# ChanTsune/Portable-Network-Archive

Measured on AMD Instinct MI355X. Metric: archive-create MiB/s (input bytes/sec), zstd-3, 10000 x 1 MiB enwik-style corpus, higher is better.
Workload: dtype u8

## Files before the change

portable-network-archive_amd/csrc/k_entropy.hip:

```cpp
#include <hip/hip_runtime.h>
#include "pna_dev.h"

namespace pna {

__constant__ uint8_t C_LL_CODE[64] = {0,1,2,3,4,5,6,7,8,9,10,11,12,13,14,15,16,16,17,17,18,18,19,19,20,20,20,20,21,21,21,21,
                                      22,22,22,22,22,22,22,22,23,23,23,23,23,23,23,23,24,24,24,24,24,24,24,24,24,24,24,24,24,24,24,24};
__constant__ uint8_t C_ML_CODE[128] = {0,1,2,3,4,5,6,7,8,9,10,11,12,13,14,15,16,17,18,19,20,21,22,23,24,25,26,27,28,29,30,31,
                                       32,32,33,33,34,34,35,35,36,36,36,36,37,37,37,37,38,38,38,38,38,38,38,38,39,39,39,39,39,39,39,39,
                                       40,40,40,40,40,40,40,40,40,40,40,40,40,40,40,40,41,41,41,41,41,41,41,41,41,41,41,41,41,41,41,41,
                                       42,42,42,42,42,42,42,42,42,42,42,42,42,42,42,42,42,42,42,42,42,42,42,42,42,42,42,42,42,42,42,42};
__constant__ uint32_t C_LL_BASE[36] = {0,1,2,3,4,5,6,7,8,9,10,11,12,13,14,15,16,18,20,22,24,28,32,40,48,64,128,256,512,1024,2048,4096,8192,16384,32768,65536};
__constant__ uint8_t  C_LL_BITS[36] = {0,0,0,0,0,0,0,0,0,0,0,0,0,0,0,0,1,1,1,1,2,2,3,3,4,6,7,8,9,10,11,12,13,14,15,16};
__constant__ uint32_t C_ML_BASE[53] = {3,4,5,6,7,8,9,10,11,12,13,14,15,16,17,18,19,20,21,22,23,24,25,26,27,28,29,30,31,32,33,34,35,37,39,41,43,47,51,59,67,83,99,131,259,515,1027,2051,4099,8195,16387,32771,65539};
__constant__ uint8_t  C_ML_BITS[53] = {0,0,0,0,0,0,0,0,0,0,0,0,0,0,0,0,0,0,0,0,0,0,0,0,0,0,0,0,0,0,0,0,1,1,1,1,2,2,3,3,4,4,5,7,8,9,10,11,12,13,14,15,16};
__constant__ int16_t C_LL_DEF[36] = {4,3,2,2,2,2,2,2,2,2,2,2,2,1,1,1,2,2,2,2,2,2,2,2,2,3,2,1,1,1,1,1,-1,-1,-1,-1};
__constant__ int16_t C_ML_DEF[53] = {1,4,3,2,2,2,2,2,2,1,1,1,1,1,1,1,1,1,1,1,1,1,1,1,1,1,1,1,1,1,1,1,1,1,1,1,1,1,1,1,1,1,1,1,1,1,-1,-1,-1,-1,-1,-1,-1};
__constant__ int16_t C_OF_DEF[29] = {1,1,1,1,1,1,2,2,2,1,1,1,1,1,1,1,1,1,1,1,1,1,1,1,-1,-1,-1,-1,-1};

__device__ __forceinline__ uint32_t hb(uint32_t v) { return 31u - (uint32_t)__builtin_clz(v); }
__device__ __forceinline__ uint32_t ll_code(uint32_t v) { return v < 64 ? C_LL_CODE[v] : hb(v) + 19; }
__device__ __forceinline__ uint32_t ml_code(uint32_t ml) { uint32_t b = ml - 3; return b < 128 ? C_ML_CODE[b] : hb(b) + 36; }

struct BitW { uint8_t *p; uint32_t pos; uint64_t acc; uint32_t nb; };
__device__ __forceinline__ void bw_init(BitW &w, uint8_t *p) { w.p = p; w.pos = 0; w.acc = 0; w.nb = 0; }
// ... 421 lines not shown
            }
        }
        for (uint32_t j = (n16 << 4) + tid; j < nlit; j += ST_THREADS) atomicAdd(&hl[bl[j]], 1u);
        const uint64_t *bs = seqs + (size_t)g * seq_cap_of(sd.blk_log);
        for (uint32_t i = tid; i < (PRE ? 0u : nseq); i += ST_THREADS) {
            const uint64_t s = bs[i];
            const uint32_t llv = seq_ll(s), mb = seq_ml(s) - 3;
            atomicAdd(&h_seq[0][tid & (HS - 1)][llv < 64 ? (uint32_t)s_llc[llv] : hb(llv) + 19], 1u);
            atomicAdd(&h_seq[1][tid & (HS - 1)][hb(seq_off(s) + 3)], 1u);
            atomicAdd(&h_seq[2][tid & (HS - 1)][mb < 128 ? (uint32_t)s_mlc[mb] : hb(mb) + 36], 1u);
        }
    }
    __syncthreads();
    if (PRE == 1) {
        const uint32_t *hs = hist + (size_t)blockIdx.x * HIST_WORDS;
        count[tid] = hs[tid];
        if (tid < 192) scount[tid >> 6][tid & 63] = hs[256 + tid];
        __syncthreads();
        for (uint32_t s = 0; s < 36; s++) nseq_seg += scount[0][s];
    } else if (PRE == 2) {
        const uint32_t *hs = hist + (size_t)blockIdx.x * HIST_WORDS;
        { uint32_t c = 0; for (uint32_t k = 0; k < HL; k++) c += h_lit[k][tid]; count[tid] = c; }
        if (tid < 192) scount[tid >> 6][tid & 63] = hs[256 + tid];
    } else {
        { uint32_t c = 0; for (uint32_t k = 0; k < HL; k++) c += h_lit[k][tid]; count[tid] = c; }
        if (tid < 192) { uint32_t w = tid >> 6, s = tid & 63, c = 0; for (uint32_t k = 0; k < HS; k++) c += h_seq[w][k][s]; scount[w][s] = c; }
    }
    __syncthreads();
    const uint32_t wave = tid >> 6, lane = tid & 63;
    if (wave != 0) {
        if (!nseq_seg) return;
        bool ok;
        if (wave == 1) ok = seq_build_wave(T, 0, scount[0], nseq_seg, 36, C_LL_DEF, 36, 6, flags, cell[1], tmp192[1], sq_sh[1], lane);
        else if (wave == 2) ok = seq_build_wave(T, 1, scount[1], nseq_seg, 32, C_OF_DEF, 29, 5, flags, cell[2], tmp192[2], sq_sh[2], lane);
        else ok = seq_build_wave(T, 2, scount[2], nseq_seg, 53, C_ML_DEF, 53, 6, flags, cell[3], tmp192[3], sq_sh[3], lane);
        if (!ok && lane == 0) atomicAnd(&T->seq_ok, 0u);
        return;
    }
    if (!(flags & F_HUF)) return;
    const int np = huf_build_lens(count, lens, order, wt, parent, hsh, lane);
    if (np < 2) return;
    uint32_t ms = 0, mb = 0;
    for (int s2 = (int)lane; s2 < 256; s2 += 64) { if (count[s2]) ms = (uint32_t)s2; const uint32_t l = lens[s2]; mb = l > mb ? l : mb; }
#pragma unroll
    for (int o = 32; o > 0; o >>= 1) { const uint32_t a2 = (uint32_t)__shfl_xor((int)ms, o), b2 = (uint32_t)__shfl_xor((int)mb, o); ms = a2 > ms ? a2 : ms; mb = b2 > mb ? b2 : mb; }
    const int max_sym = (int)ms, maxbits = (int)mb;
    if (lane < HUF_MAX + 2) { cntw_s[lane] = 0; crun_s[lane] = 0; }
    __builtin_amdgcn_wave_barrier();
    for (int s2 = (int)lane; s2 < 256; s2 += 64) { const uint32_t l = lens[s2]; if (l && s2 <= max_sym) atomicAdd(&cntw_s[(uint32_t)maxbits + 1 - l], 1u); }
    __builtin_amdgcn_wave_barrier();
    if (lane == 0) {
        uint32_t pos = 0;
        for (int w = 1; w <= maxbits; w++) { wbase_s[w] = pos; pos += cntw_s[w] << (w - 1); }
        hsh[3] = (uint32_t)max_sym; hsh[4] = (uint32_t)maxbits;
    }
    __builtin_amdgcn_wave_barrier();
    const uint64_t lane_lt = ((uint64_t)1 << lane) - 1;
    for (int r = 0; r < 4; r++) {
        const int s2 = 64 * r + (int)lane;
        const uint32_t l = (s2 <= max_sym) ? (uint32_t)lens[s2] : 0u;
        uint32_t before = 0;
        for (uint32_t L = 1; L <= (uint32_t)maxbits; L++) {
            const uint64_t m = __ballot(l == L);
            if (l == L) before = crun_s[L] + (uint32_t)__popcll(m & lane_lt);
            __builtin_amdgcn_wave_barrier();
            if (lane == 0 && m) crun_s[L] += (uint32_t)__popcll(m);
            __builtin_amdgcn_wave_barrier();
        }
        uint32_t v = 0;
        if (l) {
            const uint32_t w = (uint32_t)maxbits + 1 - l;
            v = ((wbase_s[w] + (before << (w - 1))) >> (w - 1)) | (l << 16);
        }
        T->huf_code[s2] = v;
    }
    __builtin_amdgcn_wave_barrier();
    const uint32_t tl = huf_write_tree_wave(T->tree, lens, max_sym, maxbits, wts, tmp, &wtab, cell[0], tmp192[0], sq_sh[0], lane);
    if (lane == 0) { T->tree_len = tl; T->max_sym = (uint32_t)max_sym; T->maxbits = (uint32_t)maxbits; T->huf_ok = tl > 0; }
}

constexpr uint32_t LIT_THREADS = 256;
constexpr uint32_t LIT_STAGE_Q = 184;

__global__ __launch_bounds__(LIT_THREADS)
void k_lit(const SegDesc *__restrict__ segs, const uint32_t *__restrict__ blk_seg, const uint8_t *__restrict__ lits,
           BlkInfo *__restrict__ blk, const SegTables *__restrict__ tabs, uint8_t *__restrict__ litc, uint32_t flags, uint32_t g0, uint32_t blk_log) {
    __shared__ uint32_t code[256];
    __shared__ uint32_t sbits[4];
    __shared__ unsigned long long stage[4][LIT_STAGE_Q];
    const uint32_t tid = threadIdx.x, lane = tid & 63, wave = tid >> 6;
    const uint32_t g = blockIdx.x + g0;
    const SegTables *T = tabs + blk_seg[g];
    const uint32_t nlit = blk[g].nlit;
    const uint8_t *bl = lits + ((size_t)g << blk_log);
    const uint4 *bl16 = (const uint4 *)bl;
    unsigned long long *out64 = (unsigned long long *)(litc + ((size_t)g << blk_log));
    if (!(flags & F_HUF) || nlit < 64) { if (tid == 0) { blk[g].lit_body = 0; blk[g].lit_rle = 0; } return; }
    if (!T->huf_ok) {
        const uint32_t b0 = bl[0] * 0x01010101u; int same = 1;
        const uint32_t n16 = nlit >> 4;
        for (uint32_t i = tid; i < n16; i += LIT_THREADS) { const uint4 v = bl16[i]; same &= (v.x == b0) & (v.y == b0) & (v.z == b0) & (v.w == b0); }
        for (uint32_t i = (n16 << 4) + tid; i < nlit; i += LIT_THREADS) same &= (bl[i] == (uint8_t)b0);
        same = __syncthreads_and(same);
        if (tid == 0) { blk[g].lit_rle = same ? 1u : 0u; blk[g].lit_body = 0; }
        return;
    }
    code[tid] = T->huf_code[tid];
    __syncthreads();
    const uint32_t nstreams = nlit >= 256 ? 4u : 1u;
    const uint32_t segsz = nstreams == 4 ? (nlit + 3) / 4 : nlit;
    const uint32_t a = wave * segsz;
    uint32_t m = 0;
    if (wave < nstreams) m = (nstreams == 4 && wave == 3) ? nlit - 3 * segsz : segsz;
    const uint32_t e = a + m;
    const uint32_t gfirst = a >> 4, gend = m ? (e + 15) >> 4 : gfirst;
    {
        const uint32_t b0 = bl[0];
        uint32_t bits = 0; int same = 1;
        for (uint32_t gi = gfirst + lane; gi < gend; gi += 64) {
            const uint4 v = bl16[gi];
            const uint32_t w[4] = {v.x, v.y, v.z, v.w}, base = gi << 4;
#pragma unroll
            for (uint32_t k = 0; k < 16; k++) {
                const uint32_t i = base + k, sym = (w[k >> 2] >> (8 * (k & 3))) & 0xFF;
                if (i >= a && i < e) { bits += code[sym] >> 16; same &= (sym == b0); }
            }
        }
#pragma unroll
        for (int d = 32; d >= 1; d >>= 1) bits += (uint32_t)__shfl_xor((int)bits, d);
        if (lane == 0) sbits[wave] = wave < nstreams ? bits : 0;
        same = __syncthreads_and(same);
        if (same) { if (tid == 0) { blk[g].lit_rle = 1; blk[g].lit_body = 0; } return; }
    }
    uint32_t sz[4], off[4], body = nstreams == 4 ? 6u : 0u;
    for (uint32_t k = 0; k < 4; k++) { sz[k] = k < nstreams ? (sbits[k] >> 3) + 1 : 0; off[k] = body; body += sz[k]; }
    if (tid == 0) { blk[g].lit_body = body; blk[g].lit_rle = 0; }
    if (body >= nlit || body > (1u << blk_log)) return;
    for (uint32_t i = tid; i < (body + 7) / 8; i += LIT_THREADS) out64[i] = 0;
    for (uint32_t i = lane; i < LIT_STAGE_Q; i += 64) stage[wave][i] = 0;
    __builtin_amdgcn_s_waitcnt(0);
    __syncthreads();
    if (wave < nstreams) {
        unsigned long long *st = stage[wave];
        uint32_t pos = off[wave] * 8;
        uint32_t qfl = pos >> 6;
        const uint32_t nround = (gend - gfirst + 63) / 64;
        for (uint32_t r = 0; r < nround; r++) {
            const int32_t gi = (int32_t)gend - 64 * (int32_t)(r + 1) + (int32_t)lane;
            const bool act = gi >= (int32_t)gfirst;
            unsigned long long gv[4] = {0, 0, 0, 0}; uint32_t gl[4] = {0, 0, 0, 0};
            if (act) {
                const uint4 v = bl16[gi];
                const uint32_t w[4] = {v.x, v.y, v.z, v.w}, base = (uint32_t)gi << 4;
#pragma unroll
                for (int k = 15; k >= 0; k--) {
                    const uint32_t i = base + (uint32_t)k;
                    if (i >= a && i < e) {
                        const uint32_t cv = code[(w[k >> 2] >> (8 * (k & 3))) & 0xFF];
                        const int grp = 3 - (k >> 2);
                        gv[grp] |= (unsigned long long)(cv & 0xFFFF) << gl[grp]; gl[grp] += cv >> 16;
                    }
                }
            }
            const uint32_t ltot = gl[0] + gl[1] + gl[2] + gl[3];
            uint32_t sc = ltot;
#pragma unroll
            for (int d = 1; d < 64; d <<= 1) { uint32_t t = (uint32_t)__shfl_up((int)sc, d); if (lane >= (uint32_t)d) sc += t; }
            const uint32_t rtot = (uint32_t)__shfl((int)sc, 63);
            uint32_t p = pos + (rtot - sc) - (qfl << 6);
#pragma unroll
            for (int grp = 0; grp < 4; grp++) {
                if (gl[grp]) {
                    const uint32_t qi = p >> 6, sh = p & 63;
                    atomicOr(&st[qi], gv[grp] << sh);
                    if (sh + gl[grp] > 64) atomicOr(&st[qi + 1], gv[grp] >> (64 - sh));
                    p += gl[grp];
                }
            }
            pos += rtot;
            const uint32_t nq = (pos >> 6) - qfl;
            const unsigned long long part = st[nq];
            for (uint32_t j = lane; j < nq; j += 64) { const unsigned long long x = st[j]; if (x) atomicOr(&out64[qfl + j], x); }
            for (uint32_t j = lane; j <= nq; j += 64) st[j] = (j == 0) ? part : 0ull;
            qfl += nq;
        }
        if (lane == 0) atomicOr(&st[(pos - (qfl << 6)) >> 6], 1ull << ((pos - (qfl << 6)) & 63));
        pos += 1;
        const uint32_t nq = ((pos - (qfl << 6)) + 63) >> 6;
        for (uint32_t j = lane; j < nq; j += 64) { const unsigned long long x = st[j]; if (x) atomicOr(&out64[qfl + j], x); }
    }
    if (tid == 0 && nstreams == 4) atomicOr(&out64[0], (unsigned long long)sz[0] | ((unsigned long long)sz[1] << 16) | ((unsigned long long)sz[2] << 32));
}

constexpr uint32_t SEQ_SEGS_PER_WG = 64 / BLK_PER_SEG;
static_assert(SEQ_MAX_LOG <= 8, "k_seqa: a state flush is at most 8 bits (12 are kept), the final states go into 3 x 8 bits");

constexpr uint32_t SEQA_BLKS = 21, SEQA_MAXSEG = 5;
__global__ __launch_bounds__(64)
void k_seqa(const SegDesc *__restrict__ segs, uint32_t nseg, BlkInfo *__restrict__ blk, const SegTables *__restrict__ tabs,
            uint16_t *__restrict__ seqw, uint32_t bps_log) {
    __shared__ SeqTable tab[SEQA_MAXSEG][3];
    __shared__ SeqTable ztab;
    const uint32_t lane = threadIdx.x;
    const uint32_t vb0 = blockIdx.x * SEQA_BLKS;
    const uint32_t seg0 = vb0 >> bps_log, seg1 = (vb0 + SEQA_BLKS - 1) >> bps_log;
    for (uint32_t i = lane; i < sizeof(SeqTable) / 4; i += 64) ((uint32_t *)&ztab)[i] = 0;
    for (uint32_t s = seg0; s <= seg1 && s < nseg && s - seg0 < SEQA_MAXSEG; s++) {
        const uint32_t *srcw = (const uint32_t *)&tabs[s].tab[0];
        uint32_t *dstw = (uint32_t *)&tab[s - seg0][0];
        for (uint32_t i = lane; i < 3 * sizeof(SeqTable) / 4; i += 64) dstw[i] = srcw[i];
    }
    __syncthreads();
    const uint32_t slot = lane / 3, st = lane - 3 * slot;
    const uint32_t vb = vb0 + slot;
    const uint32_t sidx = vb >> bps_log, b = vb & ((1u << bps_log) - 1);
    if (lane >= 3 * SEQA_BLKS || sidx >= nseg) return;
    const SegDesc sd = segs[sidx];
    if (b >= seg_nblk(sd)) return;
    const uint32_t g = sd.blk_base + b;
    const SegTables *T = tabs + sidx;
    const uint32_t nseq = blk[g].nseq;
    if (nseq == 0 || !T->seq_ok) { if (st == 0) blk[g].seq_bits = 0; return; }
    const uint32_t mode = T->mode[st], tlog = T->tlog[st];
    const SeqTable *tb = mode == 1 ? &ztab : &tab[sidx - seg0][st];
    const uint32_t SC = seq_cap_of(sd.blk_log);
    uint16_t *w = seqw + (size_t)g * SC * 4 + (size_t)st * SC;
    uint32_t state = 0, bits = 0;
    uint4 *w8 = (uint4 *)w;
    int32_t j = (int32_t)((nseq - 1) >> 3);
    uint4 cur = w8[j], r1 = cur, r2 = cur, r3 = cur;
    if (j > 0) r1 = w8[j - 1];
    if (j > 1) r2 = w8[j - 2];
    if (j > 2) r3 = w8[j - 3];
    bool first = true;
    for (; j >= 0; j--) {
        uint4 r4 = r3;
        if (j > 3) r4 = w8[j - 4];
        const uint32_t cw32[4] = {cur.x, cur.y, cur.z, cur.w};
        uint32_t out[4] = {0, 0, 0, 0};
        const int32_t top = (int32_t)(nseq - 1) - 8 * j;
#pragma unroll
        for (int k = 7; k >= 0; k--) {
            if (k > top) continue;
            const uint32_t cw = (cw32[k >> 1] >> (16 * (k & 1))) & 0xFFFFu;
            const SeqSym y = tb->sym[cw & 0xFF];
            uint32_t rec = 0;
            if (first) { state = y.first_state; first = false; }
            else {
                const uint32_t nb = (state + y.delta_nb) >> 16;
                rec = (state & ((1u << nb) - 1)) | (nb << 12);
                state = tb->state[(int)(state >> nb) + y.delta_find];
                bits += nb;
            }
            bits += cw >> 8;
            out[k >> 1] |= rec << (16 * (k & 1));
        }
        w8[j] = make_uint4(out[0], out[1], out[2], out[3]);
        cur = r1; r1 = r2; r2 = r3; r3 = r4;
    }
    bits += mode != 1 ? tlog : 0u;
    const uint32_t b1 = (uint32_t)__shfl((int)bits, (int)(3 * slot + 1)), b2 = (uint32_t)__shfl((int)bits, (int)(3 * slot + 2));
    atomicOr(&blk[g].pad, (state & ((1u << tlog) - 1)) << (st == 2 ? 0 : (st == 1 ? 8 : 16)));
    if (st == 0) blk[g].seq_bits = (bits + b1 + b2 + 1 + 7) >> 3;
}

template <bool GT>
__global__ __launch_bounds__(64)
void k_seq(const SegDesc *__restrict__ segs, uint32_t nseg, const uint64_t *__restrict__ seqs, BlkInfo *__restrict__ blk,
           const SegTables *__restrict__ tabs, uint8_t *__restrict__ seqc, uint32_t bps_log) {
    __shared__ SeqTable tab[GT ? 1 : SEQ_SEGS_PER_WG][3];
    __shared__ SeqTable ztab;
    __shared__ uint32_t lut_ll[64], lut_ml[128];
    __shared__ uint32_t ring[8][64];
// ... 266 lines not shown
        for (int d = 1; d < 64; d <<= 1) { const uint32_t t = (uint32_t)__shfl_up((int)incl, d); if ((int)lane >= d) incl += t; }
        if (in) { blk[g].plan = plan; blk[g].out_size = sz; blk[g].out_off = off + (incl - sz); }
        off += (uint32_t)__shfl((int)incl, 63);
    }
    if (lane == 0) seg_size[sidx] = off;
}

__global__ __launch_bounds__(1024)
void k_scan(const uint64_t *__restrict__ in, uint64_t *__restrict__ out, uint32_t n) {
    __shared__ uint64_t part[2][1024];
    const uint32_t tid = threadIdx.x;
    const uint32_t per = (n + 1023) / 1024;
    const uint32_t a = tid * per, e = a + per < n ? a + per : n;
    uint64_t s = 0;
    for (uint32_t i = a; i < e; i++) s += in[i];
    uint32_t cur = 0;
    part[0][tid] = s;
    __syncthreads();
    const uint32_t nact = per ? (n + per - 1) / per : 0;
    for (uint32_t d = 1; d < 1024 && d < nact; d <<= 1) {
        const uint64_t v = part[cur][tid] + (tid >= d ? part[cur][tid - d] : 0ull);
        part[cur ^ 1][tid] = v;
        cur ^= 1;
        __syncthreads();
    }
    uint64_t r = part[cur][tid] - s;
    if (tid == 0) out[n] = nact ? part[cur][nact - 1] : 0ull;
    for (uint32_t i = a; i < e; i++) { out[i] = r; r += in[i]; }
}

constexpr uint32_t WR_THREADS = 256;
typedef uint32_t wr_v4u __attribute__((ext_vector_type(4)));
__device__ __forceinline__ void copy_bytes(uint8_t *dst, const uint8_t *src, uint32_t n, uint32_t tid, uint32_t T) {
    const uint32_t head = (uint32_t)((16u - ((uintptr_t)dst & 15u)) & 15u), h = head < n ? head : n, mid = (n - h) >> 4;
    if (tid < h) dst[tid] = src[tid];
    for (uint32_t i = tid; i < mid; i += T) { wr_v4u v; __builtin_memcpy(&v, src + h + 16 * i, 16); *(wr_v4u *)(dst + h + 16 * i) = v; }
    for (uint32_t i = h + 16 * mid + tid; i < n; i += T) dst[i] = src[i];
}

__global__ __launch_bounds__(WR_THREADS)
void k_write(const uint8_t *__restrict__ src, const SegDesc *__restrict__ segs, const uint32_t *__restrict__ blk_seg,
             const BlkInfo *__restrict__ blk, const SegTables *__restrict__ tabs, const uint64_t *__restrict__ seg_off,
             const uint8_t *__restrict__ lits, const uint8_t *__restrict__ litc, const uint8_t *__restrict__ seqc,
             uint8_t *__restrict__ dst) {
    const uint32_t tid = threadIdx.x, g = blockIdx.x, NT = blockDim.x;
    const uint32_t sidx = blk_seg[g];
    const SegDesc sd = segs[sidx];
    const SegTables *T = tabs + sidx;
    const BlkInfo bi = blk[g];
    const uint32_t b = g - sd.blk_base;
    const uint32_t nblk = seg_nblk(sd), bsz = 1u << sd.blk_log;
    const uint32_t b0 = b * bsz, bl_len = sd.len - b0 < bsz ? sd.len - b0 : bsz;
    const bool single = (sd.first & 4) != 0;
    const uint32_t last = (b + 1 == nblk && (!single || (sd.first & 2))) ? 1u : 0u;
    uint8_t *fr = dst + seg_off[sidx];
    uint8_t *out = fr + bi.out_off;
    if (b == 0 && tid < 6 && (!single || (sd.first & 1))) { const uint8_t fh[6] = {0x28, 0xB5, 0x2F, 0xFD, 0x00, 0x50}; fr[tid] = fh[tid]; }
    const uint32_t csz = bi.out_size - 3;
    if (tid < 3) { uint32_t hdr = last | ((bi.plan & 1 ? 2u : 0u) << 1) | (csz << 3); out[tid] = (uint8_t)(hdr >> (8 * tid)); }
    out += 3;
    if (!(bi.plan & 1)) { copy_bytes(out, src + sd.src_off + b0, bl_len, tid, NT); return; }
    const uint32_t nlit = bi.nlit, nseq = bi.nseq;
    const uint8_t *bl = lits + ((size_t)g << sd.blk_log);
    uint32_t pos = 0;
    if (bi.plan & 16) {
        uint32_t h = raw_lit_hdr(nlit);
        if (tid == 0) {
            if (h == 1) out[0] = (uint8_t)(1 | (nlit << 3));
            else if (h == 2) { out[0] = (uint8_t)(1 | (1 << 2) | ((nlit & 15) << 4)); out[1] = (uint8_t)(nlit >> 4); }
            else { out[0] = (uint8_t)(1 | (3 << 2) | ((nlit & 15) << 4)); out[1] = (uint8_t)(nlit >> 4); out[2] = (uint8_t)(nlit >> 12); }
            out[h] = bl[0];
        }
        pos = h + 1;
    } else if (bi.plan & 2) {
        const uint32_t lh = 3 + (nlit >= 1024) + (nlit >= 16384), ts = (bi.plan & 4) ? T->tree_len : 0, hs = bi.lit_body;
        if (tid == 0) {
            uint64_t type = (bi.plan & 4) ? 2u : 3u, comp = ts + hs, h;
            if (lh == 3) h = type | ((uint64_t)(nlit >= 256 ? 1 : 0) << 2) | ((uint64_t)nlit << 4) | (comp << 14);
            else if (lh == 4) h = type | (2u << 2) | ((uint64_t)nlit << 4) | (comp << 18);
            else h = type | (3u << 2) | ((uint64_t)nlit << 4) | (comp << 22);
            for (uint32_t i = 0; i < lh; i++) out[i] = (uint8_t)(h >> (8 * i));
        }
        copy_bytes(out + lh, T->tree, ts, tid, NT);
        copy_bytes(out + lh + ts, litc + ((size_t)g << sd.blk_log), hs, tid, NT);
        pos = lh + ts + hs;
    } else {
        uint32_t h = raw_lit_hdr(nlit);
        if (tid == 0) {
            if (h == 1) out[0] = (uint8_t)(nlit << 3);
            else if (h == 2) { out[0] = (uint8_t)((1 << 2) | ((nlit & 15) << 4)); out[1] = (uint8_t)(nlit >> 4); }
            else { out[0] = (uint8_t)((3 << 2) | ((nlit & 15) << 4)); out[1] = (uint8_t)(nlit >> 4); out[2] = (uint8_t)(nlit >> 12); }
        }
        copy_bytes(out + h, bl, nlit, tid, NT);
        pos = h + nlit;
    }
    const uint32_t nh = nseq_hdr(nseq);
    if (tid == 0) {
        if (nh == 1) out[pos] = (uint8_t)nseq;
        else if (nh == 2) { out[pos] = (uint8_t)((nseq >> 8) + 128); out[pos + 1] = (uint8_t)nseq; }
        else { out[pos] = 255; out[pos + 1] = (uint8_t)(nseq - 0x7F00); out[pos + 2] = (uint8_t)((nseq - 0x7F00) >> 8); }
    }
    pos += nh;
    if (nseq) {
        const bool carry = (bi.plan & 8) != 0;
        if (tid == 0) {
            uint32_t m[3];
            for (int k = 0; k < 3; k++) m[k] = T->mode[k] == 0 ? 0u : (carry ? T->mode[k] : 3u);
            out[pos] = (uint8_t)((m[0] << 6) | (m[1] << 4) | (m[2] << 2));
        }
        pos += 1;
        if (carry) for (int k = 0; k < 3; k++) { copy_bytes(out + pos, T->desc[k], T->desc_len[k], tid, NT); pos += T->desc_len[k]; }
        copy_bytes(out + pos, seqc + ((size_t)g << sd.blk_log), bi.seq_bits, tid, NT);
    }
}

__global__ void k_empty(const SegDesc *__restrict__ segs, uint32_t nseg, const uint64_t *__restrict__ seg_off, uint8_t *__restrict__ dst) {
    const uint32_t sidx = blockIdx.x * blockDim.x + threadIdx.x;
    if (sidx >= nseg || segs[sidx].len != 0) return;
    const uint8_t e[9] = {0x28, 0xB5, 0x2F, 0xFD, 0x20, 0x00, 0x01, 0x00, 0x00};
    uint8_t *o = dst + seg_off[sidx];
    for (int i = 0; i < 9; i++) o[i] = e[i];
}

__global__ __launch_bounds__(1024)
void k_scan_a(const uint64_t *__restrict__ in, uint64_t *__restrict__ out, uint32_t n, uint64_t *__restrict__ chunk_sum) {
    __shared__ uint64_t part[2][1024];
    const uint32_t tid = threadIdx.x, i0 = blockIdx.x * 4096 + tid * 4;
    uint64_t v[4], s = 0;
#pragma unroll
    for (uint32_t k = 0; k < 4; k++) { v[k] = i0 + k < n ? in[i0 + k] : 0ull; s += v[k]; }
    uint32_t cur = 0;
    part[0][tid] = s;
    __syncthreads();
    for (uint32_t d = 1; d < 1024; d <<= 1) {
        part[cur ^ 1][tid] = part[cur][tid] + (tid >= d ? part[cur][tid - d] : 0ull);
        cur ^= 1;
        __syncthreads();
    }
    uint64_t r = part[cur][tid] - s;
#pragma unroll
    for (uint32_t k = 0; k < 4; k++) { if (i0 + k < n) out[i0 + k] = r; r += v[k]; }
    if (tid == 1023) chunk_sum[blockIdx.x] = part[cur][1023];
}
__global__ __launch_bounds__(1024)
void k_scan_c(uint64_t *__restrict__ out, uint32_t n, const uint64_t *__restrict__ chunk_off, uint32_t nchunk) {
    const uint32_t i0 = blockIdx.x * 4096 + threadIdx.x * 4;
    const uint64_t o = chunk_off[blockIdx.x];
#pragma unroll
    for (uint32_t k = 0; k < 4; k++) if (i0 + k < n) out[i0 + k] += o;
    if (blockIdx.x == 0 && threadIdx.x == 0) out[n] = chunk_off[nchunk];
}
void k_scan_launch(const uint64_t *in, uint64_t *out, uint32_t n, hipStream_t st) {
    hipLaunchKernelGGL(k_scan, dim3(1), dim3(1024), 0, st, in, out, n);
}
void k_scan_launch_big(const uint64_t *in, uint64_t *out, uint32_t n, hipStream_t st) {
    if (n <= 65536) { k_scan_launch(in, out, n, st); return; }
    const uint32_t nchunk = (n + 4095) / 4096;
    uint64_t *chunk_sum = out + n + 1, *chunk_off = chunk_sum + nchunk + 1;
    hipLaunchKernelGGL(k_scan_a, dim3(nchunk), dim3(1024), 0, st, in, out, n, chunk_sum);
    hipLaunchKernelGGL(k_scan, dim3(1), dim3(1024), 0, st, chunk_sum, chunk_off, nchunk);
    hipLaunchKernelGGL(k_scan_c, dim3(nchunk), dim3(1024), 0, st, out, n, chunk_off, nchunk);
}

void launch_entropy_chunk(const SegDesc *segs, uint32_t s0, uint32_t ns, const uint32_t *blk_seg, uint32_t g0, uint32_t nb,
                          const uint64_t *seqs, const uint8_t *lits, BlkInfo *blk, SegTables *tabs, uint8_t *litc, uint8_t *seqc, uint32_t *seqw,
                          uint32_t flags, uint32_t blk_log, uint32_t *hist, hipStream_t st, hipEvent_t *ev ,
                          hipStream_t side, hipEvent_t fork, hipEvent_t join, bool single_block , const uint32_t *seq_hist) {
// ... 52 lines not shown
```

portable-network-archive_amd/csrc/pna_dev.h:

```cpp
#pragma once
#include <stdint.h>
#include <stddef.h>
#include "aes_core.h"

namespace pna {

constexpr uint32_t SEG_SIZE   = 1u << 20;
#ifndef PNA_BLK_LOG
#define PNA_BLK_LOG 17
#endif
constexpr uint32_t BLK_SIZE   = 1u << PNA_BLK_LOG;
constexpr uint32_t BLK_PER_SEG = SEG_SIZE / BLK_SIZE;

constexpr uint32_t LZ_THREADS = 1024;
constexpr uint32_t LZ_WAVES   = LZ_THREADS / 64;
constexpr uint32_t TILE       = 2048;
constexpr uint32_t GROUPS_PER_WAVE = TILE / 64 / LZ_WAVES;
#ifndef LZ_HASH_ENTRIES_VALUE
#define LZ_HASH_ENTRIES_VALUE 24512
#endif
constexpr uint32_t HASH_ENTRIES = LZ_HASH_ENTRIES_VALUE;
constexpr uint32_t MIN_MATCH  = 6;
constexpr uint32_t CUT_MIN    = MIN_MATCH;
#ifndef LZ_G_ZSTD_VALUE
// ... 5 lines not shown
constexpr uint32_t NEAR_OFF   = LZ_G_ZSTD == 2 ? MAX_OFF_G2 : 65536 - 2 * 1024 * LZ_G_ZSTD - 1024 - 16 - 240;
constexpr uint32_t MAX_OFF    = 1u << 20;
constexpr uint32_t BACK_CAP   = 3;
#ifndef LZ_CAP1_VALUE
#define LZ_CAP1_VALUE 32
#endif
constexpr uint32_t CAP1       = LZ_CAP1_VALUE;
constexpr uint32_t LOOKAHEAD  = 1024;
constexpr uint32_t WIN_BYTES  = 65536;
constexpr uint32_t SEQ_CAP    = PNA_BLK_LOG == 17 ? 22528 : ((BLK_SIZE / MIN_MATCH + BLK_SIZE / 256 + 256 + 255) & ~255u);

constexpr uint32_t F_HUF = 1, F_FSE = 2, F_LAZY = 4, F_REP = 8;
constexpr uint32_t FLAG_LAZY2 = 0x400u;
constexpr uint32_t FLAG_LAZY3 = 0x800u;
constexpr uint32_t FLAG_W16 = 0x4000u;
constexpr uint32_t FLAG_LEN36 = 0x8000u;
constexpr uint32_t MAX_OFF_W3 = (1u << 19) - 1;
constexpr uint32_t FLAG_TAB3 = 0x10000u;
constexpr uint32_t SMALL_SEG = 4096, SMALL_SLOTS = 2048;
constexpr uint32_t MID_SEG = 16384, MID_SLOTS = SMALL_SLOTS;
constexpr uint32_t FLAG_T2_SHIFT = 22;
constexpr uint32_t FLAG_HAS_SMALL = 0x20000u;
constexpr uint32_t FLAG_SMALL_ONLY = 0x40000u;
constexpr uint32_t FLAG_TIER1 = 0x100000u, FLAG_TIER2 = 0x200000u;
constexpr uint32_t FLAG_ALL_SMALL = 0x80000u;
constexpr uint32_t FLAG_FAR1 = 0x1000000u;
constexpr uint32_t FLAG_STRONG2 = 0x2000000u;
constexpr uint32_t FLAG_MT_SHIFT = 28;
constexpr uint32_t FLAG_W32 = 0x2000u;
constexpr uint32_t F_FAR = 0x10, F_ADOPT = 0x20, F_INS2 = 0x40, F_STRONG = 0x80;

__host__ __device__ inline uint64_t seq_pack(uint32_t ll, uint32_t ml, uint32_t off) {
    return (uint64_t)off | ((uint64_t)ml << 20) | ((uint64_t)ll << 38);
}
__host__ __device__ inline uint32_t seq_off(uint64_t s) { return (uint32_t)(s & 0xFFFFF); }
__host__ __device__ inline uint32_t seq_ml(uint64_t s)  { return (uint32_t)((s >> 20) & 0x3FFFF); }
__host__ __device__ inline uint32_t seq_ll(uint64_t s)  { return (uint32_t)((s >> 38) & 0x3FFFF); }

struct SegDesc {
    uint64_t src_off;
    uint32_t len;
    uint32_t blk_base;
    uint32_t entry;
    uint32_t first;
    uint32_t u0, u1;
    uint32_t blk_log;
    uint32_t pad;
};
struct LzParseGrid { const SegDesc *segs_all; const uint32_t *blk_seg; uint32_t nb;
                     uint32_t *hist = nullptr; };
constexpr uint32_t BLK_LOG_MIN = 13;
static_assert(sizeof(SegDesc) == 40, "SegDesc layout");
constexpr uint32_t DRUN_CONT = 1u, DRUN_OPEN = 2u;
__host__ __device__ inline uint32_t seq_cap_of(uint32_t blk_log) {
    return blk_log >= PNA_BLK_LOG ? SEQ_CAP : ((((1u << blk_log) / MIN_MATCH + ((1u << blk_log) >> 8) + 256 + 255)) & ~255u);
}
__host__ __device__ inline uint32_t seg_nblk(const SegDesc &sd) { return (sd.len + (1u << sd.blk_log) - 1) >> sd.blk_log; }

constexpr uint32_t SEQ_MAX_LOG = 8;
struct SeqSym { uint32_t delta_nb; int16_t delta_find; uint16_t first_state; };
struct SeqTable { uint16_t state[1u << SEQ_MAX_LOG]; SeqSym sym[56]; };
struct SegTables {
    uint32_t huf_ok, tree_len, max_sym, maxbits;
    uint32_t mode[3], tlog[3], desc_len[3], seq_ok;
    uint32_t nseq_seg, pad[2], pad2;
    uint32_t huf_code[256];
    uint8_t  tree[160];
    uint8_t  desc[3][96];
    SeqTable tab[3];
};

struct BlkInfo {
    uint32_t nseq, nlit;
    uint32_t lit_body;
    uint32_t lit_rle;
    uint32_t seq_bits;
    uint32_t out_size;
    uint32_t plan;
    uint32_t pad;
    uint64_t out_off;
    uint32_t adler_a, adler_b;
};

struct DeflTables {
    uint32_t ll_code[288];
    uint32_t d_code[32];
    uint32_t hdr_bits, pad[3];
    uint8_t  hdr[400];
};

struct FrameDesc {
    uint64_t arc_off;
    uint32_t payload_len;
    uint32_t prefix_off;
    uint32_t prefix_len;
    uint32_t pad;
};
struct CrcTabs {
    uint32_t T[4][256];
    uint32_t Z[4][256];
    uint32_t sh[8];
    uint32_t pw[4][64];
};

struct CipherUnit {
    uint64_t off;
    uint64_t pos;
    uint32_t len;
    uint32_t iv_idx;
};

struct GcmEntry {
    uint64_t off;
    uint32_t len, pad;
    uint32_t h[4];
    uint32_t ej0[4];
};
struct VerdictEnt {
    uint32_t c0, c1, g0, g1, cbc_unit, pre;
};
constexpr uint32_t DIFF_TILE = 16384;
struct DiffPiece {
    uint64_t a_off, b_off, len, base;
    uint32_t entry, tile0;
};
static_assert(sizeof(DiffPiece) == 40, "DiffPiece layout");
constexpr uint32_t PICK_TILE = 16384;
struct PickPiece {
    uint64_t src_off;
    uint8_t *dst;
    uint64_t len;
    uint32_t tile0, pad;
};
static_assert(sizeof(PickPiece) == 32, "PickPiece layout");

struct ZFrame {
    uint64_t src_off;
    uint64_t dst_off;
    uint64_t src_len;
    uint64_t dst_len;
    uint32_t status;
    uint32_t out_len;
};
static_assert(sizeof(ZFrame) == 40, "ZFrame layout");

struct ZFrameX {
    uint64_t seq_base;
    uint32_t blk_base, blk_cap;
    uint32_t slot_base, slot_cap;
    uint32_t seq_cap;
    uint32_t nblk;
    uint32_t pcap, pad;
};
struct ZBlock {
    uint64_t body;
    uint64_t out_off;
    uint64_t seq_pos;
    uint32_t size, type;
    uint32_t ltype, regen, streams, lit_off, lit_csize;
    uint32_t lit_pos;
    uint32_t huf_slot, slot[3];
    uint32_t nseq, seq_off, seq_len;
    uint32_t frame, out_len, status, uses_rep;
    uint32_t pad[7];
};
static_assert(sizeof(ZBlock) == 128, "ZBlock layout");
// ... 22 lines not shown
```

Measured before the change: 145,800.

## Fuse literal Huffman size pass with encoding into fixed worst-case slot regions

The literal kernel used to run one pass to count bits per stream, then zero the output and run a second pass that encodes with global atomicOr merges. When worst-case stream sizes (from maxbits) fit in the block slot, each stream is now encoded in a single pass into its own padded region, with plain stores and no global zeroing or atomics. Stream sizes are stored in the adler fields, and the assembly stage writes the jump table and copies the four regions contiguously. The cost is one extra copy of scattered regions at assembly time, and the adler_a/adler_b fields are reused as a flag, which is fragile if nstreams is 1.

```diff
diff --git a/portable-network-archive_amd/csrc/k_entropy.hip b/portable-network-archive_amd/csrc/k_entropy.hip
--- a/portable-network-archive_amd/csrc/k_entropy.hip
+++ b/portable-network-archive_amd/csrc/k_entropy.hip
@@ -527,6 +527,58 @@
 constexpr uint32_t LIT_THREADS = 256;
 constexpr uint32_t LIT_STAGE_Q = 184;
 
+template <bool SHARED>
+__device__ __forceinline__ uint32_t lit_code_stream(const uint4 *__restrict__ bl16, const uint32_t *code, unsigned long long *st, unsigned long long *out64,
+                                                    uint32_t a, uint32_t e, uint32_t pos, uint32_t lane, uint32_t b0, int &same) {
+    const uint32_t gfirst = a >> 4, gend = (e + 15) >> 4, pos0 = pos;
+    uint32_t qfl = pos >> 6;
+    const uint32_t nround = (gend - gfirst + 63) / 64;
+    for (uint32_t r = 0; r < nround; r++) {
+        const int32_t gi = (int32_t)gend - 64 * (int32_t)(r + 1) + (int32_t)lane;
+        const bool act = gi >= (int32_t)gfirst;
+        unsigned long long gv[4] = {0, 0, 0, 0}; uint32_t gl[4] = {0, 0, 0, 0};
+        if (act) {
+            const uint4 v = bl16[gi];
+            const uint32_t w[4] = {v.x, v.y, v.z, v.w}, base = (uint32_t)gi << 4;
+#pragma unroll
+            for (int k = 15; k >= 0; k--) {
+                const uint32_t i = base + (uint32_t)k;
+                if (i >= a && i < e) {
+                    const uint32_t sym = (w[k >> 2] >> (8 * (k & 3))) & 0xFF, cv = code[sym];
+                    const int grp = 3 - (k >> 2);
+                    gv[grp] |= (unsigned long long)(cv & 0xFFFF) << gl[grp]; gl[grp] += cv >> 16;
+                    if (!SHARED) same &= (sym == b0);
+                }
+            }
+        }
+        const uint32_t ltot = gl[0] + gl[1] + gl[2] + gl[3];
+        uint32_t sc = ltot;
+#pragma unroll
+        for (int d = 1; d < 64; d <<= 1) { uint32_t t = (uint32_t)__shfl_up((int)sc, d); if (lane >= (uint32_t)d) sc += t; }
+        const uint32_t rtot = (uint32_t)__shfl((int)sc, 63);
+        uint32_t p = pos + (rtot - sc) - (qfl << 6);
+#pragma unroll
+        for (int grp = 0; grp < 4; grp++) {
+            if (gl[grp]) {
+                const uint32_t qi = p >> 6, sh = p & 63;
+                atomicOr(&st[qi], gv[grp] << sh);
+                if (sh + gl[grp] > 64) atomicOr(&st[qi + 1], gv[grp] >> (64 - sh));
+                p += gl[grp];
+            }
+        }
+        pos += rtot;
+        const uint32_t nq = (pos >> 6) - qfl;
+        const unsigned long long part = st[nq];
+        for (uint32_t j = lane; j < nq; j += 64) { const unsigned long long x = st[j]; if (SHARED) { if (x) atomicOr(&out64[qfl + j], x); } else out64[qfl + j] = x; }
+        for (uint32_t j = lane; j <= nq; j += 64) st[j] = (j == 0) ? part : 0ull;
+        qfl += nq;
+    }
+    if (lane == 0) atomicOr(&st[(pos - (qfl << 6)) >> 6], 1ull << ((pos - (qfl << 6)) & 63));
+    const uint32_t nq = ((pos + 1 - (qfl << 6)) + 63) >> 6;
+    for (uint32_t j = lane; j < nq; j += 64) { const unsigned long long x = st[j]; if (SHARED) { if (x) atomicOr(&out64[qfl + j], x); } else out64[qfl + j] = x; }
+    return pos - pos0;
+}
+
 __global__ __launch_bounds__(LIT_THREADS)
 void k_lit(const SegDesc *__restrict__ segs, const uint32_t *__restrict__ blk_seg, const uint8_t *__restrict__ lits,
            BlkInfo *__restrict__ blk, const SegTables *__restrict__ tabs, uint8_t *__restrict__ litc, uint32_t flags, uint32_t g0, uint32_t blk_log) {
@@ -539,7 +591,8 @@
     const uint32_t nlit = blk[g].nlit;
     const uint8_t *bl = lits + ((size_t)g << blk_log);
     const uint4 *bl16 = (const uint4 *)bl;
-    unsigned long long *out64 = (unsigned long long *)(litc + ((size_t)g << blk_log));
+    uint8_t *slot = litc + ((size_t)g << blk_log);
+    unsigned long long *out64 = (unsigned long long *)slot;
     if (!(flags & F_HUF) || nlit < 64) { if (tid == 0) { blk[g].lit_body = 0; blk[g].lit_rle = 0; } return; }
     if (!T->huf_ok) {
         const uint32_t b0 = bl[0] * 0x01010101u; int same = 1;
@@ -559,8 +612,24 @@
     if (wave < nstreams) m = (nstreams == 4 && wave == 3) ? nlit - 3 * segsz : segsz;
     const uint32_t e = a + m;
     const uint32_t gfirst = a >> 4, gend = m ? (e + 15) >> 4 : gfirst;
+    const uint32_t b0 = bl[0];
+    unsigned long long *st = stage[wave];
+    uint32_t roff[4];
+    if (lit_regions(nlit, T->maxbits, roff) <= (1u << blk_log)) {
+        for (uint32_t i = lane; i < LIT_STAGE_Q; i += 64) st[i] = 0;
+        __builtin_amdgcn_wave_barrier();
+        int same = 1;
+        if (wave < nstreams) sbits[wave] = lit_code_stream<false>(bl16, code, st, (unsigned long long *)(slot + roff[wave]), a, e, 0, lane, b0, same);
+        same = __syncthreads_and(same);
+        if (tid == 0) {
+            uint32_t sz[4] = {0, 0, 0, 0}, body = nstreams == 4 ? 6u : 0u;
+            for (uint32_t k = 0; k < nstreams; k++) { sz[k] = (sbits[k] >> 3) + 1; body += sz[k]; }
+            blk[g].lit_rle = same ? 1u : 0u; blk[g].lit_body = same ? 0u : body;
+            blk[g].adler_a = nstreams == 4 ? sz[0] | (sz[1] << 16) : 0u; blk[g].adler_b = sz[2] | (sz[3] << 16);
+        }
+        return;
+    }
     {
-        const uint32_t b0 = bl[0];
         uint32_t bits = 0; int same = 1;
         for (uint32_t gi = gfirst + lane; gi < gend; gi += 64) {
             const uint4 v = bl16[gi];
@@ -579,61 +648,14 @@
     }
     uint32_t sz[4], off[4], body = nstreams == 4 ? 6u : 0u;
     for (uint32_t k = 0; k < 4; k++) { sz[k] = k < nstreams ? (sbits[k] >> 3) + 1 : 0; off[k] = body; body += sz[k]; }
-    if (tid == 0) { blk[g].lit_body = body; blk[g].lit_rle = 0; }
+    if (tid == 0) { blk[g].lit_body = body; blk[g].lit_rle = 0; blk[g].adler_a = 0; blk[g].adler_b = 0; }
     if (body >= nlit || body > (1u << blk_log)) return;
     for (uint32_t i = tid; i < (body + 7) / 8; i += LIT_THREADS) out64[i] = 0;
-    for (uint32_t i = lane; i < LIT_STAGE_Q; i += 64) stage[wave][i] = 0;
+    for (uint32_t i = lane; i < LIT_STAGE_Q; i += 64) st[i] = 0;
     __builtin_amdgcn_s_waitcnt(0);
     __syncthreads();
-    if (wave < nstreams) {
-        unsigned long long *st = stage[wave];
-        uint32_t pos = off[wave] * 8;
-        uint32_t qfl = pos >> 6;
-        const uint32_t nround = (gend - gfirst + 63) / 64;
-        for (uint32_t r = 0; r < nround; r++) {
-            const int32_t gi = (int32_t)gend - 64 * (int32_t)(r + 1) + (int32_t)lane;
-            const bool act = gi >= (int32_t)gfirst;
-            unsigned long long gv[4] = {0, 0, 0, 0}; uint32_t gl[4] = {0, 0, 0, 0};
-            if (act) {
-                const uint4 v = bl16[gi];
-                const uint32_t w[4] = {v.x, v.y, v.z, v.w}, base = (uint32_t)gi << 4;
-#pragma unroll
-                for (int k = 15; k >= 0; k--) {
-                    const uint32_t i = base + (uint32_t)k;
-                    if (i >= a && i < e) {
-                        const uint32_t cv = code[(w[k >> 2] >> (8 * (k & 3))) & 0xFF];
-                        const int grp = 3 - (k >> 2);
-                        gv[grp] |= (unsigned long long)(cv & 0xFFFF) << gl[grp]; gl[grp] += cv >> 16;
-                    }
-                }
-            }
-            const uint32_t ltot = gl[0] + gl[1] + gl[2] + gl[3];
-            uint32_t sc = ltot;
-#pragma unroll
-            for (int d = 1; d < 64; d <<= 1) { uint32_t t = (uint32_t)__shfl_up((int)sc, d); if (lane >= (uint32_t)d) sc += t; }
-            const uint32_t rtot = (uint32_t)__shfl((int)sc, 63);
-            uint32_t p = pos + (rtot - sc) - (qfl << 6);
-#pragma unroll
-            for (int grp = 0; grp < 4; grp++) {
-                if (gl[grp]) {
-                    const uint32_t qi = p >> 6, sh = p & 63;
-                    atomicOr(&st[qi], gv[grp] << sh);
-                    if (sh + gl[grp] > 64) atomicOr(&st[qi + 1], gv[grp] >> (64 - sh));
-                    p += gl[grp];
-                }
-            }
-            pos += rtot;
-            const uint32_t nq = (pos >> 6) - qfl;
-            const unsigned long long part = st[nq];
-            for (uint32_t j = lane; j < nq; j += 64) { const unsigned long long x = st[j]; if (x) atomicOr(&out64[qfl + j], x); }
-            for (uint32_t j = lane; j <= nq; j += 64) st[j] = (j == 0) ? part : 0ull;
-            qfl += nq;
-        }
-        if (lane == 0) atomicOr(&st[(pos - (qfl << 6)) >> 6], 1ull << ((pos - (qfl << 6)) & 63));
-        pos += 1;
-        const uint32_t nq = ((pos - (qfl << 6)) + 63) >> 6;
-        for (uint32_t j = lane; j < nq; j += 64) { const unsigned long long x = st[j]; if (x) atomicOr(&out64[qfl + j], x); }
-    }
+    int unused = 1;
+    if (wave < nstreams) lit_code_stream<true>(bl16, code, st, out64, a, e, off[wave] * 8, lane, b0, unused);
     if (tid == 0 && nstreams == 4) atomicOr(&out64[0], (unsigned long long)sz[0] | ((unsigned long long)sz[1] << 16) | ((unsigned long long)sz[2] << 32));
 }
 
@@ -1066,7 +1088,15 @@
             for (uint32_t i = 0; i < lh; i++) out[i] = (uint8_t)(h >> (8 * i));
         }
         copy_bytes(out + lh, T->tree, ts, tid, NT);
-        copy_bytes(out + lh + ts, litc + ((size_t)g << sd.blk_log), hs, tid, NT);
+        const uint8_t *slot = litc + ((size_t)g << sd.blk_log);
+        if (bi.adler_a) {
+            const uint32_t sz[4] = {bi.adler_a & 0xFFFF, bi.adler_a >> 16, bi.adler_b & 0xFFFF, bi.adler_b >> 16};
+            uint32_t roff[4], o = lh + ts + 6;
+            lit_regions(nlit, T->maxbits, roff);
+            if (tid < 6) out[lh + ts + tid] = (uint8_t)(sz[tid >> 1] >> (8 * (tid & 1)));
+            for (uint32_t k = 0; k < 4; k++) { copy_bytes(out + o, slot + roff[k], sz[k], tid, NT); o += sz[k]; }
+        } else
+            copy_bytes(out + lh + ts, slot, hs, tid, NT);
         pos = lh + ts + hs;
     } else {
         uint32_t h = raw_lit_hdr(nlit);
diff --git a/portable-network-archive_amd/csrc/pna_dev.h b/portable-network-archive_amd/csrc/pna_dev.h
--- a/portable-network-archive_amd/csrc/pna_dev.h
+++ b/portable-network-archive_amd/csrc/pna_dev.h
@@ -111,6 +111,17 @@
     uint32_t adler_a, adler_b;
 };
 
+__host__ __device__ inline uint32_t lit_regions(uint32_t nlit, uint32_t maxbits, uint32_t off[4]) {
+    const uint32_t ns = nlit >= 256 ? 4u : 1u, segsz = ns == 4 ? (nlit + 3) / 4 : nlit;
+    uint32_t o = 0;
+    for (uint32_t k = 0; k < 4; k++) {
+        const uint32_t m = k >= ns ? 0u : (ns == 4 && k == 3) ? nlit - 3 * segsz : segsz;
+        off[k] = o;
+        if (k < ns) o += ((m * maxbits + 7) / 8 + 9 + 15) & ~15u;
+    }
+    return o;
+}
+
 struct DeflTables {
     uint32_t ll_code[288];
     uint32_t d_code[32];
```

Measured after the change: 147,800, median of 6. 1.4% higher.
